# WangFeng18/3d-gaussian-splatting

Hardware: NVIDIA H100
Metric: render+backward FPS @1080p (2.4M Gaussians) (higher is better)
Workload: dtype f32

## Files before the change

3d-gaussian-splatting_b200/csrc/bindings.cpp:

```cpp
#include <ATen/cuda/CUDAContext.h>
#include <c10/cuda/CUDACachingAllocator.h>
#include <c10/cuda/CUDAGuard.h>
#include <torch/extension.h>

#include <string>
#include <vector>

#include "../../include/gs_b200.h"

namespace gsb200 {

#define GS_CHECK_F32(x)                                                                         \
  TORCH_CHECK((x).is_cuda(), #x " must be a CUDA tensor");                                      \
  TORCH_CHECK((x).is_contiguous(), #x " must be contiguous");                                   \
  TORCH_CHECK((x).scalar_type() == at::kFloat, #x " must be float32")
#define GS_CHECK_I32(x)                                                                         \
  TORCH_CHECK((x).is_cuda(), #x " must be a CUDA tensor");                                      \
  TORCH_CHECK((x).is_contiguous(), #x " must be contiguous");                                   \
  TORCH_CHECK((x).scalar_type() == at::kInt, #x " must be int32")
#define GS_CHECK_I64(x)                                                                         \
  TORCH_CHECK((x).is_cuda(), #x " must be a CUDA tensor");                                      \
  TORCH_CHECK((x).is_contiguous(), #x " must be contiguous");                                   \
  TORCH_CHECK((x).scalar_type() == at::kLong, #x " must be int64")

// ... 890 lines not shown
        py::arg("opa_logit_min"), py::arg("delete_thresh"), py::arg("grad_thresh"), py::arg("grad_agg_max"), py::arg("tau"),
        py::arg("use_clone"), py::arg("use_split"), py::arg("clone_dt"), py::arg("generator") = py::none(),
        py::arg("feat") = py::none());
  m.def("densify_stats", &densify_stats,
        "prune / clone / split on the device from screen-space densification statistics (gs_densify_plan_stats)",
        py::arg("pos"), py::arg("rgb"), py::arg("opa"), py::arg("quat"), py::arg("scale"), py::arg("accum"),
        py::arg("count"), py::arg("max_radius"), py::arg("max_screen_px"), py::arg("scale_activation"),
        py::arg("opa_logit_min"), py::arg("delete_thresh"), py::arg("grad_thresh"), py::arg("tau"),
        py::arg("use_clone"), py::arg("use_split"), py::arg("generator") = py::none(), py::arg("feat") = py::none());
  m.def("loss_l1_ssim", &loss_l1_ssim, "fused L1 + SSIM loss, forward + image gradient (CUDA)");
  m.def("adam_step", &adam_step, "fused Adam over flat parameter / gradient buffers (CUDA)");
  m.def("tune", [](const std::string& name, int value) { check_rc(gs_tune(name.c_str(), value), "gs_tune"); },
        "set an A/B tuning knob of the blend kernels (see include/gs_b200.h gs_tune)");
  m.def("kernel_launches", []() { return (int64_t)gs_kernel_launches(); },
        "kernels of libgs_b200 launched by this process so far");
  m.attr("abi_version") = gs_abi_version();
  m.attr("SH_EVAL_PIXEL") = GS_SH_EVAL_PIXEL;
  m.attr("SH_EVAL_GAUSSIAN") = GS_SH_EVAL_GAUSSIAN;
  m.attr("FILTER2D_NONE") = GS_FILTER2D_NONE;
  m.attr("FILTER2D_DILATE") = GS_FILTER2D_DILATE;
  m.attr("FILTER2D_ANTIALIAS") = GS_FILTER2D_ANTIALIAS;
}
```

3d-gaussian-splatting_b200/csrc/blend.cu:

```cuda
#include <cstdlib>
#include <type_traits>

#include "internal.h"

namespace {

constexpr int FWD_THREADS = 64;
constexpr int FWD_PX = 4;
constexpr int FWD_STAGES = 2;

template <int FWD_CH>
struct FwdSmem {
  float4 A[FWD_STAGES][FWD_CH];
  float4 C[FWD_STAGES][FWD_CH];
  float2 B[FWD_STAGES][FWD_CH + 2];
  uint64_t full[FWD_STAGES];
};

template <typename SM, int CH>
__device__ __forceinline__ void issue_chunk(SM& sm, int stage, const float4* __restrict__ pA,
                                            const float2* __restrict__ pB, const float4* __restrict__ pC,
                                            int base, int n, int shift) {
  uint32_t bytes_a = (uint32_t)n * 16u;
  uint32_t nb = (uint32_t)(n + shift + 1) & ~1u;
// ... 7 lines not shown
template <bool GATHER>
struct StageView;
template <>
struct StageView<false> {
  const float4* A;
  const float4* C;
  const float2* B;
  __device__ __forceinline__ float4 a(int j) const { return A[j]; }
  __device__ __forceinline__ float2 b(int j) const { return B[j]; }
  __device__ __forceinline__ float4 c(int j) const { return C[j]; }
  __device__ __forceinline__ uint32_t slot(int j, int, int) const { return __float_as_uint(C[j].w); }
};
template <>
struct StageView<true> {
  const float4* R;
  int recw;
  __device__ __forceinline__ float4 a(int j) const { return R[j * recw]; }
  __device__ __forceinline__ float2 b(int j) const {
    const float4 t = R[j * recw + 1];
    return make_float2(t.x, t.y);
  }
  __device__ __forceinline__ float4 c(int j) const {
    const float4 t = R[j * recw + 1];
    return make_float4(t.z, t.w, R[j * recw + 2].x, 0.f);
  }
  __device__ __forceinline__ float depth(int j) const { return R[j * recw + 2].y; }
  __device__ __forceinline__ uint32_t slot(int j, int tx, int ty) const {
    const float4 cc = R[j * recw + 2];
    const uint32_t rxy = __float_as_uint(cc.z), rwh = __float_as_uint(cc.w);
    const uint32_t off = __float_as_uint(R[j * recw + 3].x);
    return off + ((uint32_t)ty - (rxy >> 16)) * (rwh & 0xffffu) + ((uint32_t)tx - (rxy & 0xffffu));
  }
};

template <int CH, int STAGES, int RECW>
struct GatherRing {
  float4 rec[STAGES][CH * RECW];
  uint64_t full[STAGES];
};

template <int NT, int CH>
struct GatherIds {
  uint32_t id[(CH + NT - 1) / NT];
  __device__ __forceinline__ void load(const uint32_t* __restrict__ ids, int base, int n, int tid) {
#pragma unroll
    for (int u = 0; u < (CH + NT - 1) / NT; ++u) {
      const int i = tid + u * NT;
      id[u] = i < n ? __ldg(ids + base + i) : 0u;
    }
  }
};

template <typename SM, int NT, int CH, int RECW>
__device__ __forceinline__ void gather_issue(SM& sm, int stage, const GsRec* __restrict__ grec,
                                             const uint32_t* __restrict__ goff, const GatherIds<NT, CH>& g, int n,
                                             int tid) {
#pragma unroll
  for (int u = 0; u < (CH + NT - 1) / NT; ++u) {
    const int i = tid + u * NT;
    if (i < n) {
      const float4* src = reinterpret_cast<const float4*>(grec + g.id[u]);
      const uint32_t dst = gs_smem_u32(&sm.rec[stage][i * RECW]);
#pragma unroll
      for (int q = 0; q < 3; ++q)
        asm volatile("cp.async.cg.shared.global [%0], [%1], 16;" ::"r"(dst + 16u * q), "l"(src + q) : "memory");
      if (RECW == 4)
        asm volatile("cp.async.ca.shared.global [%0], [%1], 4;" ::"r"(dst + 48u), "l"(goff + g.id[u]) : "memory");
    }
  }
  asm volatile("cp.async.mbarrier.arrive.noinc.shared::cta.b64 [%0];" ::"r"(gs_smem_u32(&sm.full[stage])) : "memory");
}

template <int FWD_CH, int PX, bool GATHER, bool AUX = false>
__global__ void __launch_bounds__(256 / PX) blend_fwd_kernel(const float4* __restrict__ pA,
                                                                 const float2* __restrict__ pB,
                                                                 const float4* __restrict__ pC,
                                                                 const GsRec* __restrict__ grec,
                                                                 const uint32_t* __restrict__ ids,
                                                                 const int* __restrict__ tile_accum, int wp, int hp,
                                                                 int ntx, float fx, float fy,
                                                                 float* __restrict__ image,
                                                                 int* __restrict__ tile_neff,
                                                                 float* __restrict__ final_img, GsCrop crop,
                                                                 GsAuxOut aux) {
  static_assert(!AUX || GATHER, "the aux outputs read |p_c| from the gathered records");
  using Smem = typename std::conditional<GATHER, GatherRing<FWD_CH, FWD_STAGES, 3>, FwdSmem<FWD_CH>>::type;
  __shared__ __align__(16) Smem sm;
  const int tile = blockIdx.x;
  const int tid = threadIdx.x;
  const int tx = tile % ntx, ty = tile / ntx;
  constexpr int FWD_PX = PX, TPR = GS_TILE / PX, NTHREADS = 256 / PX;
  const int ix0 = tx * GS_TILE + (tid % TPR) * FWD_PX;
  const int iy = ty * GS_TILE + (tid / TPR);
  float px[FWD_PX];
#pragma unroll
  for (int p = 0; p < FWD_PX; ++p) px[p] = gs_pixel_coord(ix0 + p, wp, fx);
  const float py = gs_pixel_coord(iy, hp, fy);

  const int start = tile_accum[tile];
  const int cnt = tile_accum[tile + 1] - start;
  const int shift = start & 1;
  const int nchunks = (cnt + FWD_CH - 1) / FWD_CH;

  if (tid == 0) {
    for (int s = 0; s < FWD_STAGES; ++s) gs_mbar_init(&sm.full[s], GATHER ? NTHREADS : 1);
    gs_fence_barrier_init();
  }
  __syncthreads();
  GatherIds<NTHREADS, FWD_CH> gid;
  if constexpr (GATHER) {
    for (int k = 0; k < FWD_STAGES && k < nchunks; ++k) {
      gid.load(ids, start + k * FWD_CH, min(FWD_CH, cnt - k * FWD_CH), tid);
      gather_issue<Smem, NTHREADS, FWD_CH, 3>(sm, k, grec, nullptr, gid, min(FWD_CH, cnt - k * FWD_CH), tid);
    }
    if (FWD_STAGES < nchunks) gid.load(ids, start + FWD_STAGES * FWD_CH, min(FWD_CH, cnt - FWD_STAGES * FWD_CH), tid);
  } else if (tid == 0) {
    for (int k = 0; k < FWD_STAGES && k < nchunks; ++k)
      issue_chunk<Smem, FWD_CH>(sm, k, pA, pB, pC, start + k * FWD_CH, min(FWD_CH, cnt - k * FWD_CH), shift);
  }

  float T[FWD_PX], cr[FWD_PX], cg[FWD_PX], cb[FWD_PX], dep[FWD_PX];
#pragma unroll
  for (int p = 0; p < FWD_PX; ++p) {
    T[p] = 1.f;
    cr[p] = cg[p] = cb[p] = 0.f;
    dep[p] = 0.f;
  }
  int consumed = cnt;
  int k = 0;
  for (; k < nchunks; ++k) {
    const int stage = k % FWD_STAGES;
    gs_mbar_wait(&sm.full[stage], (uint32_t)((k / FWD_STAGES) & 1));
    const int n = min(FWD_CH, cnt - k * FWD_CH);
    StageView<GATHER> sv;
    if constexpr (GATHER) {
      sv.R = sm.rec[stage];
      sv.recw = 3;
    } else {
      sv.A = sm.A[stage];
      sv.C = sm.C[stage];
      sv.B = sm.B[stage] + shift;
    }

#define GS_FWD_BODY(J)                                                                      \
  {                                                                                         \
    const float4 a = sv.a(J);                                                               \
    const float2 b = sv.b(J);                                                               \
    const float4 c = sv.c(J);                                                               \
    const float dy = py - a.y;                                                              \
    const float m1 = a.w * dy;                                                              \
    const float ev = fmaf(-b.x * dy, dy, b.y);                                              \
    float t = 0.f;                                                                          \
// ... 27 lines not shown
      for (; j < n; ++j) GS_FWD_BODY(j)
#undef GS_FWD_BODY

    bool dead = true;
#pragma unroll
    for (int p = 0; p < FWD_PX; ++p) dead = dead && !(T[p] > GS_T_STOP);
    const int all_dead = NTHREADS == 32 ? __all_sync(0xffffffffu, dead) : __syncthreads_and(dead);
    if (NTHREADS == 32) __syncwarp();
    if (all_dead) {
      consumed = min(cnt, (k + 1) * FWD_CH);
      break;
    }
    if (k + FWD_STAGES < nchunks) {
      const int kn = k + FWD_STAGES;
      if constexpr (GATHER) {
        gather_issue<Smem, NTHREADS, FWD_CH, 3>(sm, stage, grec, nullptr, gid, min(FWD_CH, cnt - kn * FWD_CH), tid);
        if (kn + 1 < nchunks) gid.load(ids, start + (kn + 1) * FWD_CH, min(FWD_CH, cnt - (kn + 1) * FWD_CH), tid);
      } else if (tid == 0)
        issue_chunk<Smem, FWD_CH>(sm, stage, pA, pB, pC, start + kn * FWD_CH, min(FWD_CH, cnt - kn * FWD_CH), shift);
    }
  }
  if (tid == 0 && k < nchunks) {
    for (int kk = k + 1; kk < nchunks && kk < k + FWD_STAGES; ++kk)
      gs_mbar_wait(&sm.full[kk % FWD_STAGES], (uint32_t)((kk / FWD_STAGES) & 1));
  }
  if constexpr (AUX) {
#pragma unroll
    for (int p = 0; p < FWD_PX; ++p) {
      cr[p] = fmaf(T[p], aux.bg[0], cr[p]);
      cg[p] = fmaf(T[p], aux.bg[1], cg[p]);
      cb[p] = fmaf(T[p], aux.bg[2], cb[p]);
// ... 409 lines not shown
    for (int p = 0; p < FWD_PX; ++p)
      gs_store_final(final_img, ix0 + p, iy, crop.left, crop.top, crop.width, crop.height, cr[p], cg[p], cb[p]);
  }
  if (tile_neff && tid == 0) tile_neff[tile] = consumed;
}

template <int PX, int STAGES_, int RQ_>
struct Bwd2Cfg {
  static constexpr int NT = 256 / PX;
  static constexpr int TPR = GS_TILE / PX;
  static constexpr int RQ = RQ_;
  static constexpr int R = NT / RQ;
  static constexpr int SQ = NT / RQ;
  static constexpr int ROWS = SQ / TPR;
  static constexpr int QS = (SQ * 6 + 31) / 32 * 32 + 32 / RQ;
  static constexpr int IS = RQ * QS + 2 - (RQ * QS) % 32 + ((RQ * QS) % 32 > 2 ? 32 : 0);
  static constexpr int STAGES = STAGES_;
};

template <int PX, int STAGES, int RQ, bool GATHER, int CH>
struct Bwd2Smem : std::conditional<GATHER, GatherRing<CH, STAGES, 4>, WsRing<STAGES>>::type {
  float part[Bwd2Cfg<PX, STAGES, RQ>::R * Bwd2Cfg<PX, STAGES, RQ>::IS];
  float pyt[GS_TILE];
  int valid[2];
};

template <int PX, int STAGES, int RQ, bool GATHER, int CH>
struct Bwd2SmemAux : Bwd2Smem<PX, STAGES, RQ, GATHER, CH> {
  static constexpr int TQS = Bwd2Cfg<PX, STAGES, RQ>::SQ, TIS = Bwd2Cfg<PX, STAGES, RQ>::NT + 1;
  static_assert(Bwd2Cfg<PX, STAGES, RQ>::NT == 32 && TQS * RQ == 32 && TIS % 32 == 1,
                "d_t plane strides are conflict free for one consumer warp only");
  float part_t[Bwd2Cfg<PX, STAGES, RQ>::R * TIS];
};

template <class Base, int R, int NT>
struct Bwd2SmemAbs : Base {
  static constexpr int AIS = NT + 1;
  static_assert(NT == 32, "absolute-gradient planes are conflict free for one consumer warp only");
// ... 38 lines not shown
    if constexpr (ABS) {
      ax += fabsf(e * fmaf(ca2, dx, -m1));
      ay += fabsf(e * fmaf(-a.w, dx, ccdy2));
    }
  }
  dst[0] = make_float2(s0, sx);
  dst[1] = make_float2(sxx, c0);
  dst[2] = make_float2(c1, c2);
  if constexpr (AUX) *dst_t = dt;
  if constexpr (ABS) {
    *dst_ax = ax;
    *dst_ay = ay;
  }
}

template <int SQ, int QS>
__device__ __forceinline__ int bwd_lane_y(int l) {
  static_assert(QS - SQ * 6 >= SQ, "a part has room for its source lanes' row y");
  return (l / SQ) * QS + SQ * 6 + l % SQ;
}

constexpr int RP_ROWLIVE = 2048, RP_SRC = RP_ROWLIVE + GS_TILE, RP_CNT = RP_SRC + 32, RP_ROW = RP_CNT + 32,
              RP_PY = RP_ROW + 32, RP_END = RP_PY + 32;
template <int PX, bool AUX, int SQ, int QS>
__device__ __forceinline__ void bwd_repack(float* __restrict__ st, const float* __restrict__ pyt, int lane, int& S,
                                           int& prow, float& py, float (&px)[PX], float (&T)[PX], float (&Rr)[PX],
                                           float (&gr)[PX], float (&gg)[PX], float (&gb)[PX], float (&gD)[PX],
                                           float (&gA)[PX]) {
  int* const rowlive = reinterpret_cast<int*>(st + RP_ROWLIVE);
  int* const lsrc = reinterpret_cast<int*>(st + RP_SRC);
  int* const lcnt = reinterpret_cast<int*>(st + RP_CNT);
  int* const lrow = reinterpret_cast<int*>(st + RP_ROW);
  float* const lpy = st + RP_PY;
  int c = 0;
#pragma unroll
  for (int p = 0; p < PX; ++p) c += T[p] > GS_T_STOP ? 1 : 0;
  if (__reduce_add_sync(0xffffffffu, c) > 16 * S) return;
  if (lane < GS_TILE) rowlive[lane] = 0;
  __syncwarp();
  if (c) atomicAdd(&rowlive[prow], c);
  __syncwarp();
  const int live = lane < GS_TILE ? rowlive[lane] : 0;
  int ns = S;
  while (ns > 1 && __reduce_add_sync(0xffffffffu, (live + ns / 2 - 1) / (ns / 2)) <= 32) ns /= 2;
  if (ns == S) return;

  int incl = c;
#pragma unroll
  for (int o = 1; o < 32; o <<= 1) {
    const int t = __shfl_up_sync(0xffffffffu, incl, o);
    if (lane >= o) incl += t;
  }
  int pos = incl - c;
#pragma unroll
  for (int p = 0; p < PX; ++p)
    if (T[p] > GS_T_STOP) {
      st[pos] = px[p];
      st[256 + pos] = T[p];
      st[512 + pos] = Rr[p];
      st[768 + pos] = gr[p];
      st[1024 + pos] = gg[p];
      st[1280 + pos] = gb[p];
      if constexpr (AUX) {
        st[1536 + pos] = gD[p];
        st[1792 + pos] = gA[p];
      }
      ++pos;
    }
  lsrc[lane] = 0;
  lcnt[lane] = 0;
  lrow[lane] = GS_TILE;
  lpy[lane] = 0.f;
  const int nl = (live + ns - 1) / ns;
  int sc = (nl << 16) | live;
#pragma unroll
  for (int o = 1; o < 32; o <<= 1) {
    const int t = __shfl_up_sync(0xffffffffu, sc, o);
    if (lane >= o) sc += t;
  }
  sc -= (nl << 16) | live;
// ... 1 lines not shown
  for (int q = 0; q < nl; ++q) {
    const int l = (sc >> 16) + q;
    lsrc[l] = (sc & 0xffff) + q * ns;
    lcnt[l] = min(ns, live - q * ns);
    lrow[l] = lane;
    lpy[l] = pyt[lane];
  }
  __syncwarp();
  const int src = lsrc[lane], n = lcnt[lane];
  prow = lrow[lane];
  py = lpy[lane];
#pragma unroll
  for (int p = 0; p < PX; ++p) {
    const bool v = p < n;
    px[p] = v ? st[src + p] : 0.f;
    T[p] = v ? st[256 + src + p] : 0.f;
    Rr[p] = v ? st[512 + src + p] : 0.f;
    gr[p] = v ? st[768 + src + p] : 0.f;
    gg[p] = v ? st[1024 + src + p] : 0.f;
    gb[p] = v ? st[1280 + src + p] : 0.f;
    if constexpr (AUX) {
      gD[p] = v ? st[1536 + src + p] : 0.f;
      gA[p] = v ? st[1792 + src + p] : 0.f;
    }
  }
  __syncwarp();
  st[bwd_lane_y<SQ, QS>(lane)] = py;
  S = ns;
}

template <int PX, bool WS, int UNR, int STAGES, int MINB, int RQ, bool GATHER, int CH, bool AUX = false,
          bool REPACK = false, bool ABS = false>
__global__ void __launch_bounds__(256 / PX + (WS ? 32 : 0), MINB)
    blend_bwd2_kernel(const float4* __restrict__ pA, const float2* __restrict__ pB, const float4* __restrict__ pC,
                      const GsRec* __restrict__ grec, const uint32_t* __restrict__ ids,
                      const uint32_t* __restrict__ goff, const int* __restrict__ tile_accum, int wp, int hp, int ntx, float fx, float fy,
                      const float* __restrict__ image, const float* __restrict__ grad_image,
                      float* __restrict__ grad_inst, int grad_is_final, GsCrop crop, uint32_t* __restrict__ row_epoch,
                      uint32_t epoch, int* __restrict__ tile_neff_b, const float* __restrict__ aux,
                      const float* __restrict__ grad_aux) {
  using Cfg = Bwd2Cfg<PX, STAGES, RQ>;
  constexpr int NT = Cfg::NT, TPR = Cfg::TPR, R = Cfg::R, SQ = Cfg::SQ, QS = Cfg::QS, IS = Cfg::IS, ROWS = Cfg::ROWS;
  static_assert(IS % 2 == 0 && QS % 2 == 0 && IS % 32 == 2 && QS % 32 == 32 / RQ, "partial buffer strides");
  static_assert(!(WS && GATHER), "the gather path issues its copies from all consumer threads");
  static_assert(GATHER || CH == WS_CH, "the packed ring is sized for CH instances per stage");
  static_assert(!AUX || GATHER, "the aux terms read |p_c| from the gathered records");
  static_assert(!REPACK || (NT == 32 && PX == 8), "the repack deals one warp's 256 pixels into slots of at most 8");
  static_assert(!REPACK || R * IS >= RP_END, "the partial buffer holds the repack's planes and tables");
  using SmemBase = typename std::conditional<AUX, Bwd2SmemAux<PX, STAGES, RQ, GATHER, CH>,
                                             Bwd2Smem<PX, STAGES, RQ, GATHER, CH>>::type;
  using Smem = typename std::conditional<ABS, Bwd2SmemAbs<SmemBase, R, NT>, SmemBase>::type;
  __shared__ __align__(16) Smem sm;
  const int tile = blockIdx.x;
  const int tid = threadIdx.x, warp = tid >> 5, lane = tid & 31;
  const int start = tile_accum[tile];
  const int cnt = tile_accum[tile + 1] - start;
  if (cnt == 0) return;
  const int nchunks = (cnt + CH - 1) / CH;
  const int tx = tile % ntx, ty = tile / ntx;
  const int shift = start & 1;
  if (tid < GS_TILE) sm.pyt[tid] = gs_pixel_coord(ty * GS_TILE + tid, hp, fy);
  if constexpr (GATHER) {
    if (tid == 0) {
      for (int s = 0; s < STAGES; ++s) gs_mbar_init(&sm.full[s], NT);
      gs_fence_barrier_init();
    }
    __syncthreads();
  } else {
    ws_init<Smem, STAGES>(sm, tid);
    if (WS) {
      if (tid >= NT) {
        if (tid == NT) ws_producer<Smem, STAGES>(sm, pA, pB, pC, start, cnt, nchunks);
        return;
      }
    } else if (tid == 0) {
      for (int k = 0; k < STAGES && k < nchunks; ++k)
        issue_chunk<Smem, CH>(sm, k, pA, pB, pC, start + k * CH, min(CH, cnt - k * CH), shift);
    }
  }
  GatherIds<NT, CH> gid;
  if constexpr (GATHER) {
    for (int k = 0; k < STAGES && k < nchunks; ++k) {
      gid.load(ids, start + k * CH, min(CH, cnt - k * CH), tid);
      gather_issue<Smem, NT, CH, 4>(sm, k, grec, goff, gid, min(CH, cnt - k * CH), tid);
    }
    if (STAGES < nchunks) gid.load(ids, start + STAGES * CH, min(CH, cnt - STAGES * CH), tid);
  }
  const int ix0 = tx * GS_TILE + (tid % TPR) * PX;
  const int iy = ty * GS_TILE + (tid / TPR);
  float px[PX];
#pragma unroll
  for (int p = 0; p < PX; ++p) px[p] = gs_pixel_coord(ix0 + p, wp, fx);
  float py = sm.pyt[tid / TPR];
  int S = PX, prow = tid / TPR;

  float T[PX], Rr[PX], gr[PX], gg[PX], gb[PX];
  {
    const size_t off = ((size_t)iy * wp + ix0) * 3;
    const float4* im = reinterpret_cast<const float4*>(image + off);
// ... 46 lines not shown
        const int x = ix0 + p - crop.left, y = iy - crop.top;
        float2 v = make_float2(0.f, 0.f);
        if (x >= 0 && x < crop.width && y >= 0 && y < crop.height)
          v = *reinterpret_cast<const float2*>(grad_aux + ((size_t)y * crop.width + x) * 2);
        gbuf[2 * p] = v.x;
        gbuf[2 * p + 1] = v.y;
      }
    }
#pragma unroll
    for (int p = 0; p < PX; ++p) {
      gD[p] = gbuf[2 * p];
      gA[p] = gbuf[2 * p + 1];
      Rr[p] = fmaf(gD[p], abuf[2 * p], fmaf(gA[p], abuf[2 * p + 1], Rr[p]));
    }
  }
  float2* const my_part = reinterpret_cast<float2*>(sm.part + (tid / SQ) * QS + (tid % SQ) * 6);
  float* my_part_t = nullptr;
  if constexpr (AUX) my_part_t = sm.part_t + (tid / SQ) * Smem::TQS + (tid % SQ);
  float *my_part_ax = nullptr, *my_part_ay = nullptr;
  if constexpr (ABS) {
    my_part_ax = sm.part_ax + tid;
    my_part_ay = sm.part_ay + tid;
  }
  const int ri = tid / RQ, rq = tid % RQ;
  const float2* const red_src = reinterpret_cast<const float2*>(sm.part + ri * IS + rq * QS);

  int consumed = cnt;
  bool finished = false;
  int k = 0;
  for (; k < nchunks && !finished; ++k) {
    const int stage = k % STAGES;
    gs_mbar_wait(&sm.full[stage], (uint32_t)((k / STAGES) & 1));
    const int n = min(CH, cnt - k * CH);
    StageView<GATHER> sv;
    if constexpr (GATHER) {
      sv.R = sm.rec[stage];
      sv.recw = 4;
    } else {
      sv.A = sm.A[stage];
      sv.C = sm.C[stage];
      sv.B = sm.B[stage] + shift;
    }

    for (int sub = 0; sub < n; sub += R) {
      const int nr = min(R, n - sub);
      auto phase1 = [&](auto np) -> int {
        constexpr int NP = decltype(np)::value, U = NP == PX ? UNR : 1;
        auto row = [&](int q) {
          float t = 0.f;
          if constexpr (AUX) t = sv.depth(sub + q);
          bwd_row<PX, AUX, NP, ABS>(sv.a(sub + q), sv.b(sub + q), sv.c(sub + q), px, py, T, Rr, gr, gg, gb,
                                    my_part + q * (IS / 2), t, &gD, &gA, AUX ? my_part_t + q * (NT + 1) : nullptr,
// ... 18 lines not shown
        if (U > 1 && !wdead)
          for (; j < nr; ++j) row(j);
        return j;
      };
      int j;
      if constexpr (REPACK) {
        switch (S) {
          case 8: j = phase1(std::integral_constant<int, 8>{}); break;
          case 4: j = phase1(std::integral_constant<int, 4>{}); break;
          case 2: j = phase1(std::integral_constant<int, 2>{}); break;
          default: j = phase1(std::integral_constant<int, 1>{}); break;
        }
      } else {
        j = phase1(std::integral_constant<int, PX>{});
      }
      bool dead = true;
#pragma unroll
      for (int p = 0; p < PX; ++p) dead = dead && !(T[p] > GS_T_STOP);
      int all_dead;
      int v0, v1;
      if (NT == 64) {
        if (lane == 0) sm.valid[warp] = j;
        all_dead = gs_bar_red_and(1, NT, dead);
        v0 = sm.valid[0];
        v1 = sm.valid[1];
      } else {
        __syncwarp();
        all_dead = __all_sync(0xffffffffu, dead);
        v0 = v1 = j;
      }
      {
        float S0 = 0.f, Sx = 0.f, Sxx = 0.f, Sy = 0.f, Sxy = 0.f, Syy = 0.f, C0 = 0.f, C1 = 0.f, C2 = 0.f;
        const bool act = ri < nr;
        float4 a = make_float4(0.f, 0.f, 0.f, 0.f);
        float2 b = make_float2(0.f, 0.f);
        if (act) {
          a = sv.a(sub + ri);
          b = sv.b(sub + ri);
        }
        const int vq = (NT == 64 && rq * SQ >= 32) ? v1 : v0;
        if (REPACK && act && ri < vq && S < PX) {
#pragma unroll
          for (int s = 0; s < SQ; ++s) {
            const float2 w0 = red_src[s * 3], w1 = red_src[s * 3 + 1], w2 = red_src[s * 3 + 2];
            float dyl = 0.f;
            if constexpr (REPACK) dyl = sm.part[bwd_lane_y<SQ, QS>(rq * SQ + s)] - a.y;
            S0 += w0.x;
            Sx += w0.y;
            Sxx += w1.x;
            C0 += w1.y;
            C1 += w2.x;
            C2 += w2.y;
            Sy = fmaf(dyl, w0.x, Sy);
            Sxy = fmaf(dyl, w0.y, Sxy);
            Syy = fmaf(dyl * dyl, w0.x, Syy);
          }
        } else if (act && ri < vq) {
#pragma unroll
          for (int r = 0; r < ROWS; ++r) {
            float2 u0 = red_src[(r * TPR) * 3], u1 = red_src[(r * TPR) * 3 + 1], u2 = red_src[(r * TPR) * 3 + 2];
#pragma unroll
// ... 47 lines not shown
          float4* out = reinterpret_cast<float4*>(grad_inst + (size_t)slot * GS_GREC);
          if (rq == 0)
            out[0] = make_float4(GS_LN2 * (2.f * a.z * Sx - a.w * Sy), GS_LN2 * (2.f * b.x * Sy - a.w * Sx),
                                 -GS_LN2 * Sxx, GS_LN2 * Sxy);
          else if (rq == 1)
            out[1] = make_float4(-GS_LN2 * Syy, GS_LN2 * S0, C0, C1);
          else if (rq == 2)
            out[2] = ABS ? make_float4(C2, Dt, GS_LN2 * Ax, GS_LN2 * Ay)
                         : make_float4(C2, Dt, 0.f, 0.f);
          else if (rq == 3 && row_epoch)
            row_epoch[slot] = epoch;
        }
      }
      if (NT == 64) gs_bar_sync(1, NT);
      else __syncwarp();
      if (all_dead) {
        consumed = min(cnt, k * CH + sub + nr);
        finished = true;
        break;
      }
      if constexpr (REPACK)
        if (S > 1) bwd_repack<PX, AUX, SQ, QS>(sm.part, sm.pyt, lane, S, prow, py, px, T, Rr, gr, gg, gb, gD, gA);
    }
    if constexpr (GATHER) {
      if (!finished && k + STAGES < nchunks) {
        const int kn = k + STAGES;
        gather_issue<Smem, NT, CH, 4>(sm, stage, grec, goff, gid, min(CH, cnt - kn * CH), tid);
        if (kn + 1 < nchunks) gid.load(ids, start + (kn + 1) * CH, min(CH, cnt - (kn + 1) * CH), tid);
      }
    } else if (tid == 0) {
      if (WS) {
        sm.consumed_chunks = k + 1;
        if (finished) sm.stop = 1;
        gs_mbar_arrive(&sm.empty[stage]);
      } else if (!finished && k + STAGES < nchunks) {
        const int kn = k + STAGES;
        issue_chunk<Smem, CH>(sm, stage, pA, pB, pC, start + kn * CH, min(CH, cnt - kn * CH), shift);
      }
    }
  }
  if (tid == 0) {
    if constexpr (!GATHER && WS) {
      gs_mbar_arrive(&sm.done);
    } else if (finished) {
      for (int kk = k; kk < nchunks && kk < k + STAGES - 1; ++kk)
        gs_mbar_wait(&sm.full[kk % STAGES], (uint32_t)((kk / STAGES) & 1));
    }
    if (tile_neff_b) tile_neff_b[tile] = consumed;
  }
  if (row_epoch || GATHER) return;
  for (int t = consumed + tid; t < cnt; t += NT) {
    const uint32_t slot = __float_as_uint(pC[start + t].w);
    float4* out = reinterpret_cast<float4*>(grad_inst + (size_t)slot * GS_GREC);
    const float4 z = make_float4(0.f, 0.f, 0.f, 0.f);
    out[0] = z;
    out[1] = z;
    out[2] = z;
  }
}

__global__ void __launch_bounds__(256) legacy_pack_kernel(const float* __restrict__ pos, const float* __restrict__ rgb,
                                                           const float* __restrict__ opa,
                                                           const float* __restrict__ cov, int m,
                                                           float4* __restrict__ pA, float2* __restrict__ pB,
// ... 126 lines not shown
                                                               g.fx, g.fy, image, tile_neff, final_img, crop, GsAuxOut{})
#define GS_FWD_CH(PX, GA)                     \
  if (ch == 64) GS_FWD_LAUNCH(64, PX, GA);    \
  else if (ch == 256) GS_FWD_LAUNCH(256, PX, GA); \
  else GS_FWD_LAUNCH(128, PX, GA)
  if (gather) {
    if (tn.fwd_px == 8) { GS_FWD_CH(8, true); } else { GS_FWD_CH(4, true); }
  } else {
    if (tn.fwd_px == 8) { GS_FWD_CH(8, false); } else { GS_FWD_CH(4, false); }
  }
#undef GS_FWD_CH
#undef GS_FWD_LAUNCH
  return cudaGetLastError();
}

cudaError_t gs_launch_blend_bwd(const float4* pA, const float2* pB, const float4* pC, const GsRec* grec,
                                const uint32_t* ids, const uint32_t* goff, const int* tile_accum, const GsFrameGeom& g,
                                const float* image,
                                const float* grad_image, float* grad_inst, int grad_is_final, const GsCrop& crop,
                                uint32_t* row_epoch, uint32_t epoch, int* tile_neff_b, cudaStream_t st,
                                const float* aux, const float* grad_aux, bool absgrad) {
  const GsTuning& tn = gs_tuning();
  const bool gather = grec != nullptr;
  if (gather && !row_epoch) return cudaErrorInvalidValue;
  if (absgrad) {
    if (!gather || (grad_aux && !aux)) return cudaErrorInvalidValue;
#define GS_BWD2_ABS(AX, RP)                                                                                        \
  blend_bwd2_kernel<8, false, 4, 3, 10, 4, true, 32, AX, RP, true><<<g.n_tiles, 32, 0, st>>>(                       \
      pA, pB, pC, grec, ids, goff, tile_accum, g.wp, g.hp, g.ntx, g.fx, g.fy, image, grad_image, grad_inst,         \
      grad_is_final, crop, row_epoch, epoch, tile_neff_b, aux, grad_aux)
// ... 13 lines not shown
    if (tn.blend_repack) GS_BWD2_AUX(true);
    else GS_BWD2_AUX(false);
#undef GS_BWD2_AUX
    return cudaGetLastError();
  }
  if (tn.bwd_kernel != 0 || gather) {
#define GS_BWD2C(PX, WS, UNR, ST, MINB, RQ, GA, CH)                                                                 \
  blend_bwd2_kernel<PX, WS, UNR, ST, MINB, RQ, GA, CH><<<g.n_tiles, 256 / PX + (WS ? 32 : 0), 0, st>>>(              \
      pA, pB, pC, grec, ids, goff, tile_accum, g.wp, g.hp, g.ntx, g.fx, g.fy, image, grad_image, grad_inst,          \
      grad_is_final,                                                                                                 \
      crop, row_epoch, epoch, tile_neff_b, nullptr, nullptr)
#define GS_BWD2(PX, WS, UNR, ST, MINB, RQ, GA) GS_BWD2C(PX, WS, UNR, ST, MINB, RQ, GA, 64)
    const int key = ((((tn.bwd_px * 10 + tn.bwd_ws) * 10 + tn.bwd_unroll) * 10 + tn.bwd_stages) * 10 + tn.bwd_rq) * 100 +
                    tn.bwd_minb;
    if (gather && tn.bwd_ch == 32) {
#define GS_BWD2_SHIPPED()                                                                                          \
  if (tn.blend_repack)                                                                                             \
    blend_bwd2_kernel<8, false, 4, 3, 10, 4, true, 32, false, true><<<g.n_tiles, 32, 0, st>>>(                      \
        pA, pB, pC, grec, ids, goff, tile_accum, g.wp, g.hp, g.ntx, g.fx, g.fy, image, grad_image, grad_inst,       \
        grad_is_final, crop, row_epoch, epoch, tile_neff_b, nullptr, nullptr);                                     \
  else                                                                                                             \
    GS_BWD2C(8, false, 4, 3, 10, 4, true, 32)
      switch (key) {
        case 8022416: GS_BWD2C(8, false, 2, 2, 16, 4, true, 32); break;
        case 8023416: GS_BWD2C(8, false, 2, 3, 16, 4, true, 32); break;
        case 8042410: GS_BWD2C(8, false, 4, 2, 10, 4, true, 32); break;
        case 8043410: GS_BWD2_SHIPPED(); break;
        default:
          if (gs_tuning().strict) return cudaErrorInvalidValue;
          GS_BWD2_SHIPPED();
          break;
      }
#undef GS_BWD2_SHIPPED
      return cudaGetLastError();
    }
    if (gather) {
      switch (key) {
        case 8012410: GS_BWD2(8, false, 1, 2, 10, 4, true); break;
        case 8022416: GS_BWD2(8, false, 2, 2, 16, 4, true); break;
        case 8022410: GS_BWD2(8, false, 2, 2, 10, 4, true); break;
        case 8042410: GS_BWD2(8, false, 4, 2, 10, 4, true); break;
        case 8023416: GS_BWD2(8, false, 2, 3, 16, 4, true); break;
        case 8012416: GS_BWD2(8, false, 1, 2, 16, 4, true); break;
        case 8012420: GS_BWD2(8, false, 1, 2, 20, 4, true); break;
        case 8012820: GS_BWD2(8, false, 1, 2, 20, 8, true); break;
        case 8013416: GS_BWD2(8, false, 1, 3, 16, 4, true); break;
        case 4012401: GS_BWD2(4, false, 1, 2, 1, 4, true); break;
        case 4042401: GS_BWD2(4, false, 4, 2, 1, 4, true); break;
// ... 63 lines not shown
  return 0;
}

int gs_blend_absgrad_supported(int d, bool gather) {
  const GsTuning& tn = gs_tuning();
  if (d != 3)
    return gs_set_error_msg(GS_ERR_UNSUPPORTED,
                            "densify statistics: absgrad needs the RGB blend (RGB or per-Gaussian SH colour); SH colour "
                            "evaluated per pixel has only grad2d");
  if (!gather)
    return gs_set_error_msg(GS_ERR_UNSUPPORTED,
                            "densify statistics: absgrad is not available on the packed path (gs_tune(\"gather\", 0))");
  if (!shipped_rgb_bwd_knobs(tn))
    return gs_set_error_msg(GS_ERR_UNSUPPORTED,
                            "densify statistics: absgrad needs the shipped backward blend knobs");
  return 0;
}

extern "C" size_t gs_draw_workspace_bytes(int m, int d) {
  if (d != 3 && gs_sh_basis_count(d) == 0) return 0;
  return legacy_ws_layout(m, d, nullptr, nullptr);
}

static int check_draw_args(const char* fn, int m, int d, int wp, int hp, int weight_normalize, int sigmoid,
                           size_t ws_bytes, void* ws) {
  if (m < 0 || wp <= 0 || hp <= 0 || (wp % GS_TILE) || (hp % GS_TILE))
    return gs_set_error_msg(GS_ERR_INVALID_ARG, fn);
  if (weight_normalize || sigmoid || (d != 3 && gs_sh_basis_count(d) == 0)) return gs_set_error_msg(GS_ERR_UNSUPPORTED, fn);
  if (m > 0 && (ws == nullptr || ws_bytes < gs_draw_workspace_bytes(m, d)))
    return gs_set_error_msg(GS_ERR_INVALID_ARG, fn);
// ... 96 lines not shown
```

include/gs_b200.h:

```cpp
#ifndef GS_B200_H
#define GS_B200_H

#include <stddef.h>
#include <stdint.h>

#ifdef __cplusplus
extern "C" {
#endif

typedef void* gs_stream_t;

#define GS_ERR_INVALID_ARG (-1)
#define GS_ERR_UNSUPPORTED (-2)
#define GS_ERR_NO_FORWARD (-3)

int gs_abi_version(void);
const char* gs_last_error(void);
int gs_tune(const char* name, int value);
unsigned long long gs_kernel_launches(void);


int gs_project_fwd(const float* pos, const float* quat, const float* scale, const float* rot,
                   const float* tran, int n, float near_plane, float half_width, float half_height,
                   float* res_pos, float* res_cov, int64_t* mask, gs_stream_t stream);

int gs_project_bwd(const float* pos, const float* quat, const float* scale, const float* rot,
                   const float* tran, const float* gradout_pos, const float* gradout_cov,
                   const int64_t* mask, int n, float* gradin_pos, float* gradin_quat,
                   float* gradin_scale, gs_stream_t stream);

int gs_tile_list(const float* pos , const float* cov , int n,
                 const float* tile_top, const float* tile_bottom, const float* tile_left,
                 const float* tile_right, int n_tiles, int* tile_n_point, int* tile_gaussian_list,
                 int max_per_tile, float thresh, int method, float tile_length_x, float tile_length_y,
// ... 203 lines not shown
```

Before: 488.2.

## Split goff into its own smem array and pad backward partials to avoid bank conflicts

```diff
diff --git a/3d-gaussian-splatting_b200/csrc/bindings.cpp b/3d-gaussian-splatting_b200/csrc/bindings.cpp
--- a/3d-gaussian-splatting_b200/csrc/bindings.cpp
+++ b/3d-gaussian-splatting_b200/csrc/bindings.cpp
@@ -928,6 +928,18 @@
         "set an A/B tuning knob of the blend kernels (see include/gs_b200.h gs_tune)");
   m.def("kernel_launches", []() { return (int64_t)gs_kernel_launches(); },
         "kernels of libgs_b200 launched by this process so far");
+  m.def("blend_bwd_profile",
+        [](c10::optional<torch::Tensor> buf) {
+          if (!buf) return check_rc(gs_blend_bwd_profile(nullptr, 0), "gs_blend_bwd_profile");
+          TORCH_CHECK(buf->is_cuda() && buf->scalar_type() == torch::kInt64 && buf->is_contiguous() && buf->dim() == 2 &&
+                          buf->size(1) == GS_BWD_PROF_FIELDS,
+                      "blend_bwd_profile: buf must be a contiguous CUDA int64 tensor [n_tiles, ", GS_BWD_PROF_FIELDS, "]");
+          check_rc(gs_blend_bwd_profile(reinterpret_cast<unsigned long long*>(buf->data_ptr<int64_t>()),
+                                        (int)buf->size(0)),
+                   "gs_blend_bwd_profile");
+        },
+        "cycle attribution of the shipped RGB backward blend into buf [n_tiles, 8] (None: off; gs_blend_bwd_profile)",
+        py::arg("buf"));
   m.attr("abi_version") = gs_abi_version();
   m.attr("SH_EVAL_PIXEL") = GS_SH_EVAL_PIXEL;
   m.attr("SH_EVAL_GAUSSIAN") = GS_SH_EVAL_GAUSSIAN;
diff --git a/3d-gaussian-splatting_b200/csrc/blend.cu b/3d-gaussian-splatting_b200/csrc/blend.cu
--- a/3d-gaussian-splatting_b200/csrc/blend.cu
+++ b/3d-gaussian-splatting_b200/csrc/blend.cu
@@ -45,29 +45,32 @@
 template <>
 struct StageView<true> {
   const float4* R;
-  int recw;
-  __device__ __forceinline__ float4 a(int j) const { return R[j * recw]; }
+  const uint32_t* G;
+  __device__ __forceinline__ float4 a(int j) const { return R[j * 3]; }
   __device__ __forceinline__ float2 b(int j) const {
-    const float4 t = R[j * recw + 1];
+    const float4 t = R[j * 3 + 1];
     return make_float2(t.x, t.y);
   }
   __device__ __forceinline__ float4 c(int j) const {
-    const float4 t = R[j * recw + 1];
-    return make_float4(t.z, t.w, R[j * recw + 2].x, 0.f);
-  }
-  __device__ __forceinline__ float depth(int j) const { return R[j * recw + 2].y; }
+    const float4 t = R[j * 3 + 1];
+    return make_float4(t.z, t.w, R[j * 3 + 2].x, 0.f);
+  }
+  __device__ __forceinline__ float depth(int j) const { return R[j * 3 + 2].y; }
   __device__ __forceinline__ uint32_t slot(int j, int tx, int ty) const {
-    const float4 cc = R[j * recw + 2];
+    const float4 cc = R[j * 3 + 2];
     const uint32_t rxy = __float_as_uint(cc.z), rwh = __float_as_uint(cc.w);
-    const uint32_t off = __float_as_uint(R[j * recw + 3].x);
-    return off + ((uint32_t)ty - (rxy >> 16)) * (rwh & 0xffffu) + ((uint32_t)tx - (rxy & 0xffffu));
+    return G[j] + ((uint32_t)ty - (rxy >> 16)) * (rwh & 0xffffu) + ((uint32_t)tx - (rxy & 0xffffu));
   }
 };
 
-template <int CH, int STAGES, int RECW>
+template <int CH, int STAGES>
 struct GatherRing {
-  float4 rec[STAGES][CH * RECW];
+  float4 rec[STAGES][CH * 3];
   uint64_t full[STAGES];
+};
+template <int CH, int STAGES>
+struct GatherRingG : GatherRing<CH, STAGES> {
+  uint32_t goff[STAGES][CH];
 };
 
 template <int NT, int CH>
@@ -82,7 +85,7 @@
   }
 };
 
-template <typename SM, int NT, int CH, int RECW>
+template <typename SM, int NT, int CH, bool GOFF>
 __device__ __forceinline__ void gather_issue(SM& sm, int stage, const GsRec* __restrict__ grec,
                                              const uint32_t* __restrict__ goff, const GatherIds<NT, CH>& g, int n,
                                              int tid) {
@@ -91,12 +94,13 @@
     const int i = tid + u * NT;
     if (i < n) {
       const float4* src = reinterpret_cast<const float4*>(grec + g.id[u]);
-      const uint32_t dst = gs_smem_u32(&sm.rec[stage][i * RECW]);
+      const uint32_t dst = gs_smem_u32(&sm.rec[stage][i * 3]);
 #pragma unroll
       for (int q = 0; q < 3; ++q)
         asm volatile("cp.async.cg.shared.global [%0], [%1], 16;" ::"r"(dst + 16u * q), "l"(src + q) : "memory");
-      if (RECW == 4)
-        asm volatile("cp.async.ca.shared.global [%0], [%1], 4;" ::"r"(dst + 48u), "l"(goff + g.id[u]) : "memory");
+      if constexpr (GOFF)
+        asm volatile("cp.async.ca.shared.global [%0], [%1], 4;" ::"r"(gs_smem_u32(&sm.goff[stage][i])),
+                     "l"(goff + g.id[u]) : "memory");
     }
   }
   asm volatile("cp.async.mbarrier.arrive.noinc.shared::cta.b64 [%0];" ::"r"(gs_smem_u32(&sm.full[stage])) : "memory");
@@ -115,7 +119,7 @@
                                                                  float* __restrict__ final_img, GsCrop crop,
                                                                  GsAuxOut aux) {
   static_assert(!AUX || GATHER, "the aux outputs read |p_c| from the gathered records");
-  using Smem = typename std::conditional<GATHER, GatherRing<FWD_CH, FWD_STAGES, 3>, FwdSmem<FWD_CH>>::type;
+  using Smem = typename std::conditional<GATHER, GatherRing<FWD_CH, FWD_STAGES>, FwdSmem<FWD_CH>>::type;
   __shared__ __align__(16) Smem sm;
   const int tile = blockIdx.x;
   const int tid = threadIdx.x;
@@ -142,7 +146,7 @@
   if constexpr (GATHER) {
     for (int k = 0; k < FWD_STAGES && k < nchunks; ++k) {
       gid.load(ids, start + k * FWD_CH, min(FWD_CH, cnt - k * FWD_CH), tid);
-      gather_issue<Smem, NTHREADS, FWD_CH, 3>(sm, k, grec, nullptr, gid, min(FWD_CH, cnt - k * FWD_CH), tid);
+      gather_issue<Smem, NTHREADS, FWD_CH, false>(sm, k, grec, nullptr, gid, min(FWD_CH, cnt - k * FWD_CH), tid);
     }
     if (FWD_STAGES < nchunks) gid.load(ids, start + FWD_STAGES * FWD_CH, min(FWD_CH, cnt - FWD_STAGES * FWD_CH), tid);
   } else if (tid == 0) {
@@ -166,7 +170,6 @@
     StageView<GATHER> sv;
     if constexpr (GATHER) {
       sv.R = sm.rec[stage];
-      sv.recw = 3;
     } else {
       sv.A = sm.A[stage];
       sv.C = sm.C[stage];
@@ -224,7 +227,7 @@
     if (k + FWD_STAGES < nchunks) {
       const int kn = k + FWD_STAGES;
       if constexpr (GATHER) {
-        gather_issue<Smem, NTHREADS, FWD_CH, 3>(sm, stage, grec, nullptr, gid, min(FWD_CH, cnt - kn * FWD_CH), tid);
+        gather_issue<Smem, NTHREADS, FWD_CH, false>(sm, stage, grec, nullptr, gid, min(FWD_CH, cnt - kn * FWD_CH), tid);
         if (kn + 1 < nchunks) gid.load(ids, start + (kn + 1) * FWD_CH, min(FWD_CH, cnt - (kn + 1) * FWD_CH), tid);
       } else if (tid == 0)
         issue_chunk<Smem, FWD_CH>(sm, stage, pA, pB, pC, start + kn * FWD_CH, min(FWD_CH, cnt - kn * FWD_CH), shift);
@@ -664,14 +667,43 @@
   static constexpr int SQ = NT / RQ;
   static constexpr int ROWS = SQ / TPR;
   static constexpr int QS = (SQ * 6 + 31) / 32 * 32 + 32 / RQ;
-  static constexpr int IS = RQ * QS + 2 - (RQ * QS) % 32 + ((RQ * QS) % 32 > 2 ? 32 : 0);
+  static constexpr bool PAIRED = NT == 32 && RQ == 4;
+  __host__ __device__ static constexpr int part_base(int q) {
+    if (!PAIRED) return q * QS;
+    int b = 0;
+    for (int i = 1; i <= q; ++i) {
+      b += SQ * 6;
+      b += (16 * (i & 1) + 8 * (i >> 1) - b % 32 + 32) % 32;
+    }
+    return b;
+  }
+  static constexpr int IS = PAIRED ? (part_base(RQ - 1) + SQ * 6 + 1) / 4 * 4 + 2
+                                   : RQ * QS + 2 - (RQ * QS) % 32 + ((RQ * QS) % 32 > 2 ? 32 : 0);
   static constexpr int STAGES = STAGES_;
 };
 
+template <class Cfg>
+__host__ __device__ constexpr bool bwd2_part_conflict_free() {
+  for (int h = 0; h < Cfg::NT; h += 16)
+    for (int v = 0; v < 3; ++v) {
+      for (int s = 0; s < Cfg::SQ; ++s) {
+        bool st[16] = {}, ld[16] = {};
+        for (int t = h; t < h + 16; ++t) {
+          const int a = (Cfg::part_base(t / Cfg::SQ) + (t % Cfg::SQ) * 6 + 2 * v) / 2 % 16;
+          const int b = ((t / Cfg::RQ) * Cfg::IS + Cfg::part_base(t % Cfg::RQ) + s * 6 + 2 * v) / 2 % 16;
+          if ((s == 0 && st[a]) || ld[b]) return false;
+          st[a] = ld[b] = true;
+        }
+      }
+    }
+  return true;
+}
+
 template <int PX, int STAGES, int RQ, bool GATHER, int CH>
-struct Bwd2Smem : std::conditional<GATHER, GatherRing<CH, STAGES, 4>, WsRing<STAGES>>::type {
+struct Bwd2Smem : std::conditional<GATHER, GatherRingG<CH, STAGES>, WsRing<STAGES>>::type {
   float part[Bwd2Cfg<PX, STAGES, RQ>::R * Bwd2Cfg<PX, STAGES, RQ>::IS];
   float pyt[GS_TILE];
+  float lane_y[32];
   int valid[2];
 };
 
@@ -740,19 +772,13 @@
   }
 }
 
-template <int SQ, int QS>
-__device__ __forceinline__ int bwd_lane_y(int l) {
-  static_assert(QS - SQ * 6 >= SQ, "a part has room for its source lanes' row y");
-  return (l / SQ) * QS + SQ * 6 + l % SQ;
-}
-
-constexpr int RP_ROWLIVE = 2048, RP_SRC = RP_ROWLIVE + GS_TILE, RP_CNT = RP_SRC + 32, RP_ROW = RP_CNT + 32,
-              RP_PY = RP_ROW + 32, RP_END = RP_PY + 32;
-template <int PX, bool AUX, int SQ, int QS>
-__device__ __forceinline__ void bwd_repack(float* __restrict__ st, const float* __restrict__ pyt, int lane, int& S,
-                                           int& prow, float& py, float (&px)[PX], float (&T)[PX], float (&Rr)[PX],
-                                           float (&gr)[PX], float (&gg)[PX], float (&gb)[PX], float (&gD)[PX],
-                                           float (&gA)[PX]) {
+constexpr int RP_PLANE = 128, RP_ROWLIVE = 8 * RP_PLANE, RP_SRC = RP_ROWLIVE + GS_TILE, RP_CNT = RP_SRC + 32,
+              RP_ROW = RP_CNT + 32, RP_PY = RP_ROW + 32, RP_END = RP_PY + 32;
+template <int PX, bool AUX>
+__device__ __forceinline__ void bwd_repack(float* __restrict__ st, const float* __restrict__ pyt,
+                                           float* __restrict__ lane_y, int lane, int& S, int& prow, float& py,
+                                           float (&px)[PX], float (&T)[PX], float (&Rr)[PX], float (&gr)[PX],
+                                           float (&gg)[PX], float (&gb)[PX], float (&gD)[PX], float (&gA)[PX]) {
   int* const rowlive = reinterpret_cast<int*>(st + RP_ROWLIVE);
   int* const lsrc = reinterpret_cast<int*>(st + RP_SRC);
   int* const lcnt = reinterpret_cast<int*>(st + RP_CNT);
@@ -782,14 +808,14 @@
   for (int p = 0; p < PX; ++p)
     if (T[p] > GS_T_STOP) {
       st[pos] = px[p];
-      st[256 + pos] = T[p];
-      st[512 + pos] = Rr[p];
-      st[768 + pos] = gr[p];
-      st[1024 + pos] = gg[p];
-      st[1280 + pos] = gb[p];
+      st[RP_PLANE + pos] = T[p];
+      st[2 * RP_PLANE + pos] = Rr[p];
+      st[3 * RP_PLANE + pos] = gr[p];
+      st[4 * RP_PLANE + pos] = gg[p];
+      st[5 * RP_PLANE + pos] = gb[p];
       if constexpr (AUX) {
-        st[1536 + pos] = gD[p];
-        st[1792 + pos] = gA[p];
+        st[6 * RP_PLANE + pos] = gD[p];
+        st[7 * RP_PLANE + pos] = gA[p];
       }
       ++pos;
     }
@@ -821,23 +847,48 @@
   for (int p = 0; p < PX; ++p) {
     const bool v = p < n;
     px[p] = v ? st[src + p] : 0.f;
-    T[p] = v ? st[256 + src + p] : 0.f;
-    Rr[p] = v ? st[512 + src + p] : 0.f;
-    gr[p] = v ? st[768 + src + p] : 0.f;
-    gg[p] = v ? st[1024 + src + p] : 0.f;
-    gb[p] = v ? st[1280 + src + p] : 0.f;
+    T[p] = v ? st[RP_PLANE + src + p] : 0.f;
+    Rr[p] = v ? st[2 * RP_PLANE + src + p] : 0.f;
+    gr[p] = v ? st[3 * RP_PLANE + src + p] : 0.f;
+    gg[p] = v ? st[4 * RP_PLANE + src + p] : 0.f;
+    gb[p] = v ? st[5 * RP_PLANE + src + p] : 0.f;
     if constexpr (AUX) {
-      gD[p] = v ? st[1536 + src + p] : 0.f;
-      gA[p] = v ? st[1792 + src + p] : 0.f;
-    }
-  }
+      gD[p] = v ? st[6 * RP_PLANE + src + p] : 0.f;
+      gA[p] = v ? st[7 * RP_PLANE + src + p] : 0.f;
+    }
+  }
+  lane_y[lane] = py;
   __syncwarp();
-  st[bwd_lane_y<SQ, QS>(lane)] = py;
   S = ns;
 }
 
+enum { BP_SETUP, BP_WAIT, BP_PHASE1, BP_PHASE2, BP_REPACK, BP_ISSUE, BP_TAIL, BP_ROUNDS };
+static_assert(BP_ROUNDS + 1 == GS_BWD_PROF_FIELDS, "profile fields");
+__device__ unsigned long long* g_bwd2_prof;
+template <bool ON>
+struct Bwd2Prof {
+  __device__ __forceinline__ void lap(int) {}
+  __device__ __forceinline__ void round() {}
+  __device__ __forceinline__ void store(int, int) {}
+};
+template <>
+struct Bwd2Prof<true> {
+  uint32_t t = (uint32_t)clock();
+  uint32_t acc[GS_BWD_PROF_FIELDS] = {};
+  __device__ __forceinline__ void lap(int f) {
+    const uint32_t n = (uint32_t)clock();
+    acc[f] += n - t;
+    t = n;
+  }
+  __device__ __forceinline__ void round() { ++acc[BP_ROUNDS]; }
+  __device__ __forceinline__ void store(int tile, int tid) {
+    if (tid == 0)
+      for (int f = 0; f < GS_BWD_PROF_FIELDS; ++f) g_bwd2_prof[(size_t)tile * GS_BWD_PROF_FIELDS + f] = acc[f];
+  }
+};
+
 template <int PX, bool WS, int UNR, int STAGES, int MINB, int RQ, bool GATHER, int CH, bool AUX = false,
-          bool REPACK = false, bool ABS = false>
+          bool REPACK = false, bool ABS = false, bool PROF = false>
 __global__ void __launch_bounds__(256 / PX + (WS ? 32 : 0), MINB)
     blend_bwd2_kernel(const float4* __restrict__ pA, const float2* __restrict__ pB, const float4* __restrict__ pC,
                       const GsRec* __restrict__ grec, const uint32_t* __restrict__ ids,
@@ -848,7 +899,9 @@
                       const float* __restrict__ grad_aux) {
   using Cfg = Bwd2Cfg<PX, STAGES, RQ>;
   constexpr int NT = Cfg::NT, TPR = Cfg::TPR, R = Cfg::R, SQ = Cfg::SQ, QS = Cfg::QS, IS = Cfg::IS, ROWS = Cfg::ROWS;
-  static_assert(IS % 2 == 0 && QS % 2 == 0 && IS % 32 == 2 && QS % 32 == 32 / RQ, "partial buffer strides");
+  static_assert(Cfg::PAIRED ? bwd2_part_conflict_free<Cfg>()
+                            : IS % 2 == 0 && QS % 2 == 0 && IS % 32 == 2 && QS % 32 == 32 / RQ,
+                "partial buffer strides");
   static_assert(!(WS && GATHER), "the gather path issues its copies from all consumer threads");
   static_assert(GATHER || CH == WS_CH, "the packed ring is sized for CH instances per stage");
   static_assert(!AUX || GATHER, "the aux terms read |p_c| from the gathered records");
@@ -863,6 +916,7 @@
   const int start = tile_accum[tile];
   const int cnt = tile_accum[tile + 1] - start;
   if (cnt == 0) return;
+  Bwd2Prof<PROF> prof;
   const int nchunks = (cnt + CH - 1) / CH;
   const int tx = tile % ntx, ty = tile / ntx;
   const int shift = start & 1;
@@ -889,7 +943,7 @@
   if constexpr (GATHER) {
     for (int k = 0; k < STAGES && k < nchunks; ++k) {
       gid.load(ids, start + k * CH, min(CH, cnt - k * CH), tid);
-      gather_issue<Smem, NT, CH, 4>(sm, k, grec, goff, gid, min(CH, cnt - k * CH), tid);
+      gather_issue<Smem, NT, CH, true>(sm, k, grec, goff, gid, min(CH, cnt - k * CH), tid);
     }
     if (STAGES < nchunks) gid.load(ids, start + STAGES * CH, min(CH, cnt - STAGES * CH), tid);
   }
@@ -966,7 +1020,7 @@
       Rr[p] = fmaf(gD[p], abuf[2 * p], fmaf(gA[p], abuf[2 * p + 1], Rr[p]));
     }
   }
-  float2* const my_part = reinterpret_cast<float2*>(sm.part + (tid / SQ) * QS + (tid % SQ) * 6);
+  float2* const my_part = reinterpret_cast<float2*>(sm.part + Cfg::part_base(tid / SQ) + (tid % SQ) * 6);
   float* my_part_t = nullptr;
   if constexpr (AUX) my_part_t = sm.part_t + (tid / SQ) * Smem::TQS + (tid % SQ);
   float *my_part_ax = nullptr, *my_part_ay = nullptr;
@@ -975,19 +1029,21 @@
     my_part_ay = sm.part_ay + tid;
   }
   const int ri = tid / RQ, rq = tid % RQ;
-  const float2* const red_src = reinterpret_cast<const float2*>(sm.part + ri * IS + rq * QS);
+  const float2* const red_src = reinterpret_cast<const float2*>(sm.part + ri * IS + Cfg::part_base(rq));
 
   int consumed = cnt;
   bool finished = false;
   int k = 0;
+  prof.lap(BP_SETUP);
   for (; k < nchunks && !finished; ++k) {
     const int stage = k % STAGES;
     gs_mbar_wait(&sm.full[stage], (uint32_t)((k / STAGES) & 1));
+    prof.lap(BP_WAIT);
     const int n = min(CH, cnt - k * CH);
     StageView<GATHER> sv;
     if constexpr (GATHER) {
       sv.R = sm.rec[stage];
-      sv.recw = 4;
+      sv.G = sm.goff[stage];
     } else {
       sv.A = sm.A[stage];
       sv.C = sm.C[stage];
@@ -1036,6 +1092,8 @@
       } else {
         j = phase1(std::integral_constant<int, PX>{});
       }
+      prof.lap(BP_PHASE1);
+      prof.round();
       bool dead = true;
 #pragma unroll
       for (int p = 0; p < PX; ++p) dead = dead && !(T[p] > GS_T_STOP);
@@ -1066,7 +1124,7 @@
           for (int s = 0; s < SQ; ++s) {
             const float2 w0 = red_src[s * 3], w1 = red_src[s * 3 + 1], w2 = red_src[s * 3 + 2];
             float dyl = 0.f;
-            if constexpr (REPACK) dyl = sm.part[bwd_lane_y<SQ, QS>(rq * SQ + s)] - a.y;
+            if constexpr (REPACK) dyl = sm.lane_y[rq * SQ + s] - a.y;
             S0 += w0.x;
             Sx += w0.y;
             Sxx += w1.x;
@@ -1144,18 +1202,20 @@
       }
       if (NT == 64) gs_bar_sync(1, NT);
       else __syncwarp();
+      prof.lap(BP_PHASE2);
       if (all_dead) {
         consumed = min(cnt, k * CH + sub + nr);
         finished = true;
         break;
       }
       if constexpr (REPACK)
-        if (S > 1) bwd_repack<PX, AUX, SQ, QS>(sm.part, sm.pyt, lane, S, prow, py, px, T, Rr, gr, gg, gb, gD, gA);
+        if (S > 1) bwd_repack<PX, AUX>(sm.part, sm.pyt, sm.lane_y, lane, S, prow, py, px, T, Rr, gr, gg, gb, gD, gA);
+      prof.lap(BP_REPACK);
     }
     if constexpr (GATHER) {
       if (!finished && k + STAGES < nchunks) {
         const int kn = k + STAGES;
-        gather_issue<Smem, NT, CH, 4>(sm, stage, grec, goff, gid, min(CH, cnt - kn * CH), tid);
+        gather_issue<Smem, NT, CH, true>(sm, stage, grec, goff, gid, min(CH, cnt - kn * CH), tid);
         if (kn + 1 < nchunks) gid.load(ids, start + (kn + 1) * CH, min(CH, cnt - (kn + 1) * CH), tid);
       }
     } else if (tid == 0) {
@@ -1168,6 +1228,7 @@
         issue_chunk<Smem, CH>(sm, stage, pA, pB, pC, start + kn * CH, min(CH, cnt - kn * CH), shift);
       }
     }
+    prof.lap(BP_ISSUE);
   }
   if (tid == 0) {
     if constexpr (!GATHER && WS) {
@@ -1178,6 +1239,8 @@
     }
     if (tile_neff_b) tile_neff_b[tile] = consumed;
   }
+  prof.lap(BP_TAIL);
+  prof.store(tile, tid);
   if (row_epoch || GATHER) return;
   for (int t = consumed + tid; t < cnt; t += NT) {
     const uint32_t slot = __float_as_uint(pC[start + t].w);
@@ -1334,6 +1397,11 @@
   return cudaGetLastError();
 }
 
+static struct {
+  unsigned long long* buf;
+  int n_tiles;
+} s_bwd_prof = {nullptr, 0};
+
 cudaError_t gs_launch_blend_bwd(const float4* pA, const float2* pB, const float4* pC, const GsRec* grec,
                                 const uint32_t* ids, const uint32_t* goff, const int* tile_accum, const GsFrameGeom& g,
                                 const float* image,
@@ -1377,8 +1445,16 @@
     const int key = ((((tn.bwd_px * 10 + tn.bwd_ws) * 10 + tn.bwd_unroll) * 10 + tn.bwd_stages) * 10 + tn.bwd_rq) * 100 +
                     tn.bwd_minb;
     if (gather && tn.bwd_ch == 32) {
+#define GS_BWD2_PROF(RP)                                                                                           \
+  blend_bwd2_kernel<8, false, 4, 3, 10, 4, true, 32, false, RP, false, true><<<g.n_tiles, 32, 0, st>>>(             \
+      pA, pB, pC, grec, ids, goff, tile_accum, g.wp, g.hp, g.ntx, g.fx, g.fy, image, grad_image, grad_inst,         \
+      grad_is_final, crop, row_epoch, epoch, tile_neff_b, nullptr, nullptr)
 #define GS_BWD2_SHIPPED()                                                                                          \
-  if (tn.blend_repack)                                                                                             \
+  if (s_bwd_prof.buf) {                                                                                            \
+    if (s_bwd_prof.n_tiles < g.n_tiles) return cudaErrorInvalidValue;                                              \
+    if (tn.blend_repack) GS_BWD2_PROF(true);                                                                       \
+    else GS_BWD2_PROF(false);                                                                                      \
+  } else if (tn.blend_repack)                                                                                      \
     blend_bwd2_kernel<8, false, 4, 3, 10, 4, true, 32, false, true><<<g.n_tiles, 32, 0, st>>>(                      \
         pA, pB, pC, grec, ids, goff, tile_accum, g.wp, g.hp, g.ntx, g.fx, g.fy, image, grad_image, grad_inst,       \
         grad_is_final, crop, row_epoch, epoch, tile_neff_b, nullptr, nullptr);                                     \
@@ -1395,6 +1471,7 @@
           break;
       }
 #undef GS_BWD2_SHIPPED
+#undef GS_BWD2_PROF
       return cudaGetLastError();
     }
     if (gather) {
@@ -1488,6 +1565,15 @@
   if (!shipped_rgb_bwd_knobs(tn))
     return gs_set_error_msg(GS_ERR_UNSUPPORTED,
                             "densify statistics: absgrad needs the shipped backward blend knobs");
+  return 0;
+}
+
+extern "C" int gs_blend_bwd_profile(unsigned long long* buf, int n_tiles) {
+  if (buf && n_tiles <= 0) return gs_set_error_msg(GS_ERR_INVALID_ARG, "gs_blend_bwd_profile: n_tiles must be > 0");
+  if (cudaMemcpyToSymbol(g_bwd2_prof, &buf, sizeof(buf)) != cudaSuccess)
+    return gs_set_error_msg(GS_ERR_INVALID_ARG, "gs_blend_bwd_profile: cannot set the profiling buffer");
+  s_bwd_prof.buf = buf;
+  s_bwd_prof.n_tiles = buf ? n_tiles : 0;
   return 0;
 }
 
diff --git a/include/gs_b200.h b/include/gs_b200.h
--- a/include/gs_b200.h
+++ b/include/gs_b200.h
@@ -18,6 +18,8 @@
 const char* gs_last_error(void);
 int gs_tune(const char* name, int value);
 unsigned long long gs_kernel_launches(void);
+#define GS_BWD_PROF_FIELDS 8
+int gs_blend_bwd_profile(unsigned long long* buf, int n_tiles);
 
 
 int gs_project_fwd(const float* pos, const float* quat, const float* scale, const float* rot,
```

Result: no change. 491.5 (median of 6 runs) (+0.7%).
